# gear-genomics/tracy

Hardware: AMD Instinct MI355X
Metric: GCUPS (tracy align: Gotoh affine-gap DP cells per second, whole job) (higher is better)
Workload: dtype int16 (score sweeps) / int32 (tracebacks)

## Files before the change

### tracy_amd/csrc/pipe_kernels.h

```cpp
#ifndef TRACY_AMD_PIPE_KERNELS_H
#define TRACY_AMD_PIPE_KERNELS_H

#include <hip/hip_runtime.h>

#include "capi_internal.h"
#include "stream_plan.h"

namespace {
using namespace tracyhip;

__global__ __launch_bounds__(64) void trim_kernel(const uint8_t* __restrict__ ops, const uint64_t* __restrict__ ops_off,
                                                  const uint32_t* __restrict__ ops_len, const uint32_t* __restrict__ ref_len,
                                                  const uint8_t* __restrict__ forward, const uint32_t* __restrict__ trim_left,
                                                  const uint32_t* __restrict__ trim_right, uint32_t ntraces, TrimRec* __restrict__ out) {
  const uint32_t t = blockIdx.x;
  if (t >= ntraces) return;
  const uint8_t* o = ops + ops_off[t];
  const uint32_t L = ops_len[t];
  const uint32_t lane = threadIdx.x;
  int32_t s = -1, e = -1;
  for (uint32_t base = 0; base < L; base += 64) {
    const uint32_t j = base + lane;
    const bool hit = (j < L) && (o[L - 1 - j] != 'h');
    const unsigned long long m = __ballot(hit);
// ... 106 lines not shown
    float pr[5];
    for (int k = 0; k < 5; ++k) pr[k] = prof[d.off + (uint64_t)k * d.stride + r];
    int32_t best = INT32_MIN;
    for (uint32_t b = 0; b < 5; ++b) {
      const int32_t q = onehot_score(pr, b, fmatch, fmis);
      best = q > best ? q : best;
    }
    sum += best > 0 ? best : 0;
    sum1 += best > -1 ? best : -1;
  }
  for (int o = 32; o > 0; o >>= 1) { sum += __shfl_down(sum, o, 64); sum1 += __shfl_down(sum1, o, 64); }
  if (threadIdx.x == 0) {
    out[blockIdx.x] = sum;
    if (out1) out1[blockIdx.x] = sum1;
  }
}

constexpr uint32_t kCqBytesPerThread = 16;
__global__ void encode_cq_kernel(const uint8_t* __restrict__ in, uint8_t* __restrict__ out, uint64_t n, int32_t* flag, uint8_t* __restrict__ special) {
  const uint64_t i0 = ((uint64_t)blockIdx.x * blockDim.x + threadIdx.x) * kCqBytesPerThread;
  int32_t f = 0;
  if (i0 < n) {
    const uint32_t cnt = n - i0 < kCqBytesPerThread ? (uint32_t)(n - i0) : kCqBytesPerThread;
    uint8_t b[kCqBytesPerThread];
    if (cnt == kCqBytesPerThread) __builtin_memcpy(b, in + i0, kCqBytesPerThread);
    else for (uint32_t j = 0; j < cnt; ++j) b[j] = in[i0 + j];
    bool any = false;
#pragma unroll
    for (uint32_t j = 0; j < kCqBytesPerThread; ++j) {
      const uint32_t c = j < cnt ? cq_code(b[j]) : 0u;
      b[j] = (uint8_t)c;
      if (c >= 4u) { f |= c >= 5u ? 2 : 4; any = true; }
    }
    if (cnt == kCqBytesPerThread) __builtin_memcpy(out + i0, b, kCqBytesPerThread);
    else for (uint32_t j = 0; j < cnt; ++j) out[i0 + j] = b[j];
    if (any && special) { special[i0 >> 8] = 1; special[(i0 + cnt - 1) >> 8] = 1; }
  }
  if (f) atomicOr(flag, f);
}
__global__ void cq_rows_kernel(const uint8_t* __restrict__ in, uint64_t n, int32_t* flag) {
  const uint64_t i0 = ((uint64_t)blockIdx.x * blockDim.x + threadIdx.x) * kCqBytesPerThread;
  if (i0 >= n) return;
  const uint32_t cnt = n - i0 < kCqBytesPerThread ? (uint32_t)(n - i0) : kCqBytesPerThread;
  uint8_t b[kCqBytesPerThread];
  if (cnt == kCqBytesPerThread) __builtin_memcpy(b, in + i0, kCqBytesPerThread);
  else for (uint32_t j = 0; j < cnt; ++j) b[j] = in[i0 + j];
  bool bad = false;
#pragma unroll
  for (uint32_t j = 0; j < kCqBytesPerThread; ++j)
    if (j < cnt && !cq_row_char(b[j])) bad = true;
  if (bad) atomicOr(flag, 1);
}

__device__ __forceinline__ uint32_t encode_word(uint32_t w, uint32_t cnt, bool& any_special, bool& invalid) {
  uint32_t codes = 0;
#pragma unroll
  for (uint32_t j = 0; j < 4u; ++j) {
    const uint8_t ch = (uint8_t)(w >> (8 * j));
    const uint8_t up = ch & 0xdfu;
    const uint32_t c = up == 'A' ? 0u : up == 'C' ? 1u : up == 'G' ? 2u : up == 'T' ? 3u : up == 'N' ? 4u : 5u;
    if (j < cnt) {
      invalid |= !(ch == 'A' || ch == 'C' || ch == 'G' || ch == 'T' || ch == 'N');
      any_special |= c >= 4u;
    }
    codes |= c << (8 * j);
  }
  return codes;
}
__global__ __launch_bounds__(256) void encode_codes_kernel(const uint8_t* __restrict__ in, uint8_t* __restrict__ out, uint64_t n,
                                                           uint8_t* __restrict__ special, int32_t* __restrict__ verr) {
  const uint64_t i0 = ((uint64_t)blockIdx.x * blockDim.x + threadIdx.x) * 16u;
  if (i0 >= n) return;
  bool any_special = false, invalid = false;
  if (n - i0 >= 16u) {
    uint32_t w[4];
    __builtin_memcpy(w, in + i0, 16);
#pragma unroll
    for (int q = 0; q < 4; ++q) w[q] = encode_word(w[q], 4u, any_special, invalid);
    __builtin_memcpy(out + i0, w, 16);
  } else {
    for (uint64_t i = i0; i < n; i += 4) {
      const uint32_t cnt = (n - i < 4u) ? (uint32_t)(n - i) : 4u;
      uint32_t w = 0;
      for (uint32_t j = 0; j < cnt; ++j) w |= (uint32_t)in[i + j] << (8 * j);
      const uint32_t c = encode_word(w, cnt, any_special, invalid);
      for (uint32_t j = 0; j < cnt; ++j) out[i + j] = (uint8_t)(c >> (8 * j));
    }
  }
  if (any_special) special[i0 >> 8] = 1;
  if (verr && invalid) atomicOr(verr, 4);
}

struct VoteDesc { uint64_t a1_off, a2_off; uint32_t stride, m, n, pad; };
constexpr int kVoteK = 11;
constexpr uint32_t kVoteBits = 1u << 16;
constexpr uint32_t kVotePiece = 65, kVoteTile = 64 * kVotePiece;
__device__ inline uint32_t vote_hash(uint32_t kmer) { return (kmer * 0x9E3779B1u) >> 16; }
__global__ __launch_bounds__(64) void kmer_vote_kernel(const VoteDesc* __restrict__ desc, const float* __restrict__ prof,
                                                       const uint8_t* __restrict__ codes, uint32_t* __restrict__ votes) {
  __shared__ uint32_t bm[2][kVoteBits / 32];
  __shared__ uint8_t cons[1040];
  __shared__ __attribute__((aligned(16))) uint8_t win[kVoteTile + 16];
  const VoteDesc d = desc[blockIdx.x];
  const uint32_t lane = threadIdx.x;
  uint32_t hf = 0, hr = 0;
  const uint32_t m = d.m < 1024u ? d.m : 1024u;
  if (m >= (uint32_t)kVoteK && d.n >= (uint32_t)kVoteK) {
    for (uint32_t i = lane; i < kVoteBits / 32; i += 64) { bm[0][i] = 0; bm[1][i] = 0; }
    constexpr uint32_t kCols = 8;
    for (uint32_t j0 = 0; j0 < m; j0 += 64 * kCols) {
      float v[kCols][4];
#pragma unroll
      for (uint32_t u = 0; u < kCols; ++u) {
        const uint32_t j = j0 + 64 * u + lane, jc = j < m ? j : m - 1;
#pragma unroll
        for (uint32_t k = 0; k < 4; ++k) v[u][k] = prof[d.a1_off + (uint64_t)k * d.stride + jc];
      }
#pragma unroll
      for (uint32_t u = 0; u < kCols; ++u) {
        const uint32_t j = j0 + 64 * u + lane;
        uint32_t best = 0;
        float bv = v[u][0];
#pragma unroll
        for (uint32_t k = 1; k < 4; ++k) {
          const bool g = v[u][k] > bv;
          bv = g ? v[u][k] : bv;
          best = g ? k : best;
        }
        if (j < m) cons[j] = (uint8_t)best;
      }
    }
    __syncthreads();
// ... 64 lines not shown
```

### tracy_amd/csrc/pipeline.hip

```cpp
#include <hip/hip_runtime.h>

#include <algorithm>
#include <cstdlib>
#include <cstring>
#include <numeric>
#include <string>
#include <thread>
#include <vector>

#include "../../include/tracy_hip.h"
#include "capi_internal.h"
#include "launch.h"
#include "pipe_internal.h"
#include "pipe_kernels.h"
#include "stream_fields.h"

using namespace tracyhip;

namespace {
void reset_call_stats(tracyhip_ctx* ctx, uint32_t ntraces) {
  ctx->stats = tracyhip_call_stats{};
  ctx->stats.traces = ntraces;
  for (auto* l : ctx->lanes) l->stats = tracyhip_call_stats{};
}
// ... 689 lines not shown
  if ((rc = ctx_begin(ctx))) return rc;
  *empty = job->ntraces == 0;
  return TRACYHIP_OK;
}

static int align_traces_one(tracyhip_ctx* ctx, const tracyhip_align_job* job, const tracyhip_params* prm, int mem, const tracyhip_align_result* out) {
  bool empty = false;
  int rc = align_check_args(ctx, job, prm, mem, out, &empty);
  if (rc || empty) return rc;
  if (job->refs.kind == TRACYHIP_SEQ_PROFILE) return wildtype_align(ctx, job, prm, mem, out);
  rc = stream_align(ctx, job, prm, mem, out);
  if (rc != kStreamNo) return rc;
  return align_traces_legacy(ctx, job, prm, mem, out);
}

struct AlignRun {
  tracyhip_ctx* ctx;
  const tracyhip_align_job* job;
  const tracyhip_params* prm;
  const int mem;
  const tracyhip_align_result* out;
  const uint32_t nt;
  const tracyhip_seqset& sp;
  const tracyhip_seqset& sr;
  hipStream_t st;
  tracyhip_params p;
  const void *d_prof = nullptr, *d_ref = nullptr;
  int32_t* d_verr = nullptr;
  std::vector<uint32_t> mf, mt, tl, rn, ridx;
  const TrimSrc trims;
  std::vector<B16TableDesc> td;
  bool b16 = false;
  OrientOut oo;
  std::vector<TrimRec> h_trim;
  void *d_final_sc = nullptr, *d_ops = nullptr, *d_olen = nullptr;
  uint64_t ops_total = 0;

  AlignRun(tracyhip_ctx* c, const tracyhip_align_job* j, const tracyhip_params* q, int m, const tracyhip_align_result* o)
      : ctx(c), job(j), prm(q), mem(m), out(o), nt(j->ntraces), sp(j->profiles), sr(j->refs), st(c->stream), p(*q), trims(trims_of(j)) {
    p.hfree = 1;
    p.vfree = 0;
  }

  int setup() {
    int rc;
    const uint64_t ep = seqset_extent(sp), er = seqset_extent(sr);
    if ((rc = stage_in(ctx, ctx->dev[DB_IN1], sp.data, ep * 4, mem, &d_prof))) return rc;
    if ((rc = stage_in(ctx, ctx->dev[DB_IN2], sr.data, er, mem, &d_ref))) return rc;
    HIP_TRY(ctx->dev[DB_ERR].ensure(kErrBytes));
    HIP_TRY(hipMemsetAsync(ctx->dev[DB_ERR].p, 0, kErrBytes, st));
    d_verr = static_cast<int32_t*>(ctx->dev[DB_ERR].p) + kErrVerdictWord;
    HIP_TRY(ctx->ensure_codes(er ? er : 1, st));
    if (er) {
      hipLaunchKernelGGL(encode_codes_kernel, dim3((unsigned)((er + 4095) / 4096)), dim3(256), 0, st, static_cast<const uint8_t*>(d_ref),
                         ctx->codes(), er, ctx->special_blocks(), job->oriented ? (int32_t*)nullptr : d_verr);
      HIP_TRY(hipGetLastError());
    }
    mf.resize(nt); mt.resize(nt); tl.resize(nt); rn.resize(nt); ridx.resize(nt);
    uint64_t max_mn = 0;
    for (uint32_t t = 0; t < nt; ++t) {
      ridx[t] = job->ref_index ? job->ref_index[t] : t;
      if (ridx[t] >= sr.count) return set_error(TRACYHIP_ERR_ARG, "ref_index[%u] out of range", t);
      mf[t] = sp.length[t];
      rn[t] = sr.length[ridx[t]];
      uint32_t l = trims.left(t), r = trims.right(t);
      if ((uint64_t)l + r >= mf[t]) { l = 0; r = 0; }
      tl[t] = l;
      mt[t] = mf[t] - (l + r);
      max_mn = std::max<uint64_t>(max_mn, (uint64_t)mf[t] + rn[t]);
    }
    if ((rc = check_params(&p, max_mn))) return rc;

    return TRACYHIP_OK;
  }

  int orient() {
    int rc;
    std::vector<uint64_t> off1(nt);
    uint64_t tot1 = 0;
    for (uint32_t t = 0; t < nt; ++t) { off1[t] = tot1; tot1 += (uint64_t)mt[t] + rn[t]; }
    OrientIn oi{};
    HIP_TRY(ensure_into(ctx->dev[DB_PRELIM_OPS], tot1 ? tot1 : 1, oi.d_ops));
    HIP_TRY(ensure_into(ctx->dev[DB_PRELIM_OFF], nt, oi.d_ops_off));
    HIP_TRY(ensure_into(ctx->dev[DB_PRELIM_LEN], nt, oi.d_ops_len));
    HIP_TRY(ensure_into(ctx->dev[DB_PRELIM_SCORE], nt, oi.d_score));
    HIP_TRY(ctx->pin[PB_TMP].ensure(sizeof(uint64_t) * (size_t)nt + (size_t)nt * 16));
    std::memcpy(ctx->pin[PB_TMP].p, off1.data(), sizeof(uint64_t) * (size_t)nt);
    HIP_TRY(hipMemcpyAsync(ctx->dev[DB_PRELIM_OFF].p, ctx->pin[PB_TMP].p, sizeof(uint64_t) * (size_t)nt, hipMemcpyHostToDevice, st));
    std::vector<uint64_t> a1o(nt), a2o(nt);
    for (uint32_t t = 0; t < nt; ++t) { a1o[t] = sp.offset[t] + tl[t]; a2o[t] = sr.offset[ridx[t]]; }
    b16 = p.ge < 0 && p.go <= 0 && sub_limit(&p) <= kWideScore && !ctx->knobs.no_band16;
    if (b16) {
      td.resize(nt);
      for (uint32_t t = 0; t < nt; ++t) td[t] = B16TableDesc{sp.offset[t], 0, mf[t], mf[t], 0, 0};
      if ((rc = build_b16_tables(ctx, ctx->dev[DB_B16TAB_PROFILE], d_prof, false, td, &p))) return rc;
    }
    oi.nt = nt; oi.d_prof = d_prof; oi.a1_off = a1o.data(); oi.mf = mf.data(); oi.mt = mt.data(); oi.a2_off = a2o.data(); oi.rn = rn.data();
    oi.oriented = job->oriented; oi.exact = job->strand_by_certificate == 0; oi.d_verr = d_verr; oi.ends_only = true;
    if (b16) { oi.d_qp = static_cast<const int16_t*>(ctx->dev[DB_B16TAB_PROFILE].p); oi.td = td.data(); oi.row0 = tl.data(); }
    if ((rc = orient_and_align(ctx, p, oi, oo))) return rc;

    return TRACYHIP_OK;
  }

  int trim() {
    HIP_TRY(ctx->dev[DB_TRIMREC].ensure(sizeof(TrimRec) * (size_t)nt));
    HIP_TRY(ctx->dev[DB_TRIM_IN].ensure(3 * sizeof(uint32_t) * (size_t)nt + (size_t)nt));
// ... 512 lines not shown
      if ((uint64_t)(uint32_t)(TL + TR + 1) >= (uint64_t)mf[t]) { soff[t] = 0; sl[t] = mf[t]; }
      else { soff[t] = TL; sl[t] = mf[t] - TL - TR; }
      max_mn = std::max<uint64_t>(max_mn, (uint64_t)mf[t] + rn[t]);
      maxbc = std::max(maxbc, mf[t]);
      maxcol = std::max(maxcol, mt[t]);
    }
    if ((rc = check_params(&p, max_mn))) return rc;

    ep = seqset_extent(sp); er = seqset_extent(sr);
    for (uint32_t t = 0; t < nt; ++t) {
      if (!bc.peaks) sext = std::max<uint64_t>(sext, bc.signal_offset[t] + 4ull * bc.nsamples[t]);
      bext = std::max<uint64_t>(bext, bc.bc_offset[t] + bc.bc_len[t]);
    }
    if ((rc = stage_in(ctx, buf(), sp.data, ep * 4, mem, &d_prof))) return rc;
    if ((rc = stage_in(ctx, buf(), sr.data, er, mem, &d_ref))) return rc;
    if (wildtype && given && (rc = stage_in(ctx, buf(), srp.data, seqset_extent(srp) * 4, mem, &d_refprof))) return rc;
    if (wildtype && !given) {
      wt_rev_base = seqset_extent(srp);
      DevBuf& bw = buf();
      float* d_w; HIP_TRY(ensure_into(bw, std::max<uint64_t>(2 * wt_rev_base, 1), d_w));
      HIP_TRY(hipMemcpyAsync(d_w, srp.data, wt_rev_base * 4, mem == TRACYHIP_MEM_HOST ? hipMemcpyHostToDevice : hipMemcpyDeviceToDevice, st));
      std::vector<ProfSeq> hs(srp.count);
      for (uint32_t i = 0; i < srp.count; ++i) hs[i] = ProfSeq{srp.offset[i], srp.length[i], 0};
      const ProfSeq* ds;
      if ((rc = upload(ctx, buf(), hs, &ds))) return rc;
      HIP_TRY(launch_prof_revcomp(ds, srp.count, d_w, d_w, wt_rev_base, st));
      d_refprof = d_w;
    }
    if (bc.peaks) { if ((rc = stage_in(ctx, buf(), bc.peaks, bext * 16, mem, &d_peaks))) return rc; }
    else {
      if ((rc = stage_in(ctx, buf(), bc.signal, sext * 4, mem, &d_sig))) return rc;
      if ((rc = stage_in(ctx, buf(), bc.bcpos, bext * 4, mem, &d_pos))) return rc;
    }
    for (uint32_t t = 0; t < nt; ++t) dext = std::max<uint64_t>(dext, out->dcp_offset[t] + 2ull * dp.maxindel + 2);
    if ((rc = io(bc.primary, bext, true, &d_pri))) return rc;
    if ((rc = io(bc.secondary, bext, true, &d_sec))) return rc;
    if ((rc = io(out->bp, sizeof(BreakpointOut) * (size_t)nt, false, &d_bp))) return rc;
    if ((rc = io(out->secdecomp, bext, false, &d_sd))) return rc;
    if ((rc = io(out->fractions, sizeof(double) * 2 * (size_t)nt, false, &d_fr))) return rc;
    if ((rc = io(out->dcp_indel, dext * 4, false, &d_di))) return rc;
    if ((rc = io(out->dcp_err, dext * 4, false, &d_de))) return rc;
    if (mem == TRACYHIP_MEM_HOST) {
      HIP_TRY(hipMemsetAsync(d_di, 0, dext * 4, st));
      HIP_TRY(hipMemsetAsync(d_de, 0, dext * 4, st));
    }
    if ((rc = io(out->dstatus, sizeof(DecompOut) * (size_t)nt, false, &d_dst))) return rc;
    if ((rc = io(out->score_trim, sizeof(int32_t) * (size_t)nt, false, &d_strim))) return rc;

    HIP_TRY(ctx->dev[DB_ERR].ensure(kErrBytes));
    HIP_TRY(hipMemsetAsync(ctx->dev[DB_ERR].p, 0, kErrBytes, st));
    HIP_TRY(ctx->ensure_codes(er ? er : 1, st));
    if (er) {
      int32_t* d_verr = static_cast<int32_t*>(ctx->dev[DB_ERR].p) + kErrVerdictWord;
      hipLaunchKernelGGL(encode_codes_kernel, dim3((unsigned)((er + 4095) / 4096)), dim3(256), 0, st, static_cast<const uint8_t*>(d_ref),
                         ctx->codes(), er, ctx->special_blocks(), job->oriented ? (int32_t*)nullptr : d_verr);
      HIP_TRY(hipGetLastError());
      int32_t herr = 0;
      HIP_TRY(hipMemcpyAsync(&herr, d_verr, sizeof(int32_t), hipMemcpyDeviceToHost, st));
      HIP_TRY(ctx_sync(ctx));
      if ((herr & 4) && !wildtype) return set_error(TRACYHIP_ERR_ARG, "reference windows must be upper-case [ACGTN] (loadSingleFasta, fasta.h:54-95)");
    }

    return TRACYHIP_OK;
  }

  int orientation() {
    int rc;
    stage_clock.mark("decompose.2_orientation");
    HIP_TRY(b_sc2.ensure(sizeof(int32_t) * 2 * (size_t)nt));
    h_sc2.assign(2 * (size_t)nt, 0);
    if (!given && !shared_stages) {
      DpProblem pb;
      DpProblemLease lease(ctx, pb);
      pb.mode = MODE_PROF; pb.a1_profile = true; pb.a2_profile = true; pb.d_a1 = d_prof; pb.d_a2 = d_refprof;
      pb.desc.resize(2 * (size_t)nt); pb.k.resize(2 * (size_t)nt);
      for (uint32_t t = 0; t < nt; ++t) {
        PairDesc d = qp_desc(t, true);
        d.a2_off = srp.offset[ridx[t]];
        pb.desc[t] = d;
        d.out = nt + t; d.a2_off += wt_rev_base;
        pb.desc[nt + t] = d;
        pb.k[t] = pb.k[nt + t] = choose_k(d.m, MODE_PROF);
      }
      if ((rc = run_dp(ctx, pb, &p, false, false, static_cast<int32_t*>(b_sc2.p), nullptr, nullptr, nullptr))) return rc;
      HIP_TRY(hipMemcpy(h_sc2.data(), b_sc2.p, sizeof(int32_t) * 2 * (size_t)nt, hipMemcpyDeviceToHost));
    }
    h_fwd.assign(nt, 0); h_rc.assign(nt, 0);
    if (!shared_stages)
      for (uint32_t t = 0; t < nt; ++t) {
        if (given) { h_fwd[t] = job->oriented[t] ? 1 : 0; h_rc[t] = 0; }
        else { h_fwd[t] = h_sc2[t] > h_sc2[nt + t] ? 1 : 0; h_rc[t] = !h_fwd[t]; }
      }

    return TRACYHIP_OK;
  }

  int gotoh_rows() {
    int rc;
    stage_clock.mark("decompose.3_gotoh");
    off1.resize(nt);
    for (uint32_t t = 0; t < nt; ++t) { off1[t] = tot1; tot1 += (uint64_t)mt[t] + rn[t]; }
    HIP_TRY(b_ops1.ensure(tot1 ? tot1 : 1));
    HIP_TRY(b_len1.ensure(sizeof(uint32_t) * (size_t)nt));
    HIP_TRY(b_r0.ensure(tot1 ? tot1 : 1));
    HIP_TRY(b_r1.ensure(tot1 ? tot1 : 1));
    if ((rc = upload(ctx, buf(), off1, &d_off1))) return rc;
    if (shared_stages) {
// ... 838 lines not shown
```

### tracy_amd/csrc/stream.hip

```cpp
#include <hip/hip_runtime.h>

#include <algorithm>
#include <cstring>
#include <numeric>
#include <string>
#include <type_traits>
#include <vector>

#include "../../include/tracy_hip.h"
#include "capi_internal.h"
#include "decompose_launch.h"
#include "launch.h"
#include "pipe_internal.h"
#include "pipe_kernels.h"
#include "stream_fields.h"
#include "stream_plan.h"

using namespace tracyhip;

#define TRY(expr) do { const int _rc = (expr); if (_rc) return _rc; } while (0)

namespace {

struct Arena {
// ... 198 lines not shown
    d.a2_off = G.ref_off; d.n = G.rn; d.a2_stride = G.rn;
    d.out = t;
    d.flags = S.rc ? PAIR_A2_REVCOMP : 0u;
    desc_trim[t] = d;
  }
  });
}

__global__ void s_prelim_plan_kernel(SParams p, int mode, int early, const SGeom* __restrict__ geom, STrace* __restrict__ tr, const uint32_t* __restrict__ d_ce,
                                     const int32_t* __restrict__ top, uint32_t* __restrict__ dead, PairDesc* __restrict__ cand,
                                     uint8_t* __restrict__ kc, int prio) {
  wave_prio(prio);
  const uint32_t t = blockIdx.x * blockDim.x + threadIdx.x;
  if (t >= p.nt) return;
  kc[t] = 0;
  STrace S = tr[t];
  if (((S.mark & ST_EARLY) != 0u) != (early != 0)) return;
  if (dead[t]) return;
  const SGeom G = geom[t];
  const bool from_front = S.cls == 0 && S.rc == S.g;
  const uint32_t ce = from_front ? S.ce : d_ce[t];
  S.ce = ce;
  uint32_t dd = 0;
  if (ce == 0u) dd = SD_JUNK;
  else {
    const SubWindow sw = s_sub_window(G.mt, ce, top[t], S.sstar, p.ge);
    S.gap = (uint32_t)(sw.g < 0x7fffffff ? sw.g : 0x7fffffff);
    S.shift = sw.a;
    int K = sw.K;
    if (K && mode == 0 && !b16_origin_ok(p.match, p.mismatch, p.go, p.ge, G.mt, sw.n)) K = 0;
    if (K && !s_fits_lds(sw.n, K)) K = 0;
    if (!K) dd = SD_PRELIM_BAND;
    else if (sw.n > p.ncap) dd = SD_SHAPE;
    else {
      PairDesc q{};
      q.a1_off = G.tab_off + G.tl;
      q.a1_stride = G.tab_stride;
      q.m = G.mt;
      q.n = sw.n;
      q.a2_stride = sw.n;
      q.a2_off = G.ref_off + (S.rc ? (uint64_t)(G.rn - ce) : (uint64_t)sw.a);
      q.flags = S.rc ? PAIR_A2_REVCOMP : 0u;
      q.out = t;
      q.ckpt_off = band_pack(sw.dlo, sw.dhi);
      q.lastrow_off = mode == 0 ? 0ull : ((uint64_t)(G.rn - ce) | ((uint64_t)sw.a << 32));
      cand[t] = q;
      kc[t] = (uint8_t)K;
    }
  }
  tr[t] = S;
  if (dd) dead[t] |= dd;
}

constexpr uint32_t kScanBlock = 256, kScanTop = 1024;
struct ScanPart { uint32_t n[4]; unsigned long long bytes; };
__device__ __forceinline__ int s_bucket(int K, const PairDesc& d, int quads) {
  return K == 12 ? 0 : K == 8 ? 1 : (quads && b16_narrow_ok(band_dmin(d), band_dmax(d))) ? 3 : 2;
}
__device__ __forceinline__ unsigned long long s_word_bytes(const PairDesc& d, int K, int kind, unsigned long long* words = nullptr) {
  if (words) *words = b16_words(d.m, d.n, K, band_dmin(d), band_dmax(d));
  return kind == 0 ? ((b16_store_words(d.m, d.n, K, band_dmin(d), band_dmax(d)) * b16_word_bytes(K) + 15ull) & ~15ull) : 0ull;
}
__global__ __launch_bounds__(kScanBlock) void s_scan_partial_kernel(const PairDesc* __restrict__ cand, const uint8_t* __restrict__ kc, uint32_t n, int kind,
                                                                    int quads, ScanPart* __restrict__ part, int prio) {
  wave_prio(prio);
  __shared__ uint32_t s_n[4];
  __shared__ unsigned long long s_b;
  if (threadIdx.x < 4) s_n[threadIdx.x] = 0;
  if (threadIdx.x == 4) s_b = 0;
  __syncthreads();
  const uint32_t i = blockIdx.x * kScanBlock + threadIdx.x;
  const int K = i < n ? kc[i] : 0;
  if (K) {
    const PairDesc d = cand[i];
    atomicAdd(&s_n[s_bucket(K, d, quads)], 1u);
    if (kind == 0) atomicAdd(&s_b, s_word_bytes(d, K, kind));
  }
  __syncthreads();
  if (threadIdx.x == 0) part[blockIdx.x] = ScanPart{{s_n[0], s_n[1], s_n[2], s_n[3]}, s_b};
}
__global__ __launch_bounds__(kScanTop) void s_scan_top_kernel(ScanPart* __restrict__ part, uint32_t nb, uint32_t* __restrict__ count,
                                                              unsigned long long* __restrict__ stat, int prio) {
  wave_prio(prio);
  __shared__ uint32_t s_n[4][kScanTop];
  __shared__ unsigned long long s_b[kScanTop];
  const uint32_t tid = threadIdx.x;
  const uint32_t per = (nb + kScanTop - 1) / kScanTop;
  const uint32_t lo = tid * per < nb ? tid * per : nb, hi = lo + per < nb ? lo + per : nb;
  uint32_t c[4] = {0, 0, 0, 0};
  unsigned long long bytes = 0;
  for (uint32_t i = lo; i < hi; ++i) { for (int b = 0; b < 4; ++b) c[b] += part[i].n[b]; bytes += part[i].bytes; }
  for (int b = 0; b < 4; ++b) s_n[b][tid] = c[b];
  s_b[tid] = bytes;
  __syncthreads();
  for (uint32_t d = 1; d < kScanTop; d <<= 1) {
    uint32_t v[4] = {0, 0, 0, 0};
    unsigned long long vb = 0;
    if (tid >= d) { for (int b = 0; b < 4; ++b) v[b] = s_n[b][tid - d]; vb = s_b[tid - d]; }
    __syncthreads();
    for (int b = 0; b < 4; ++b) s_n[b][tid] += v[b];
    s_b[tid] += vb;
    __syncthreads();
  }
  uint32_t at[4];
  for (int b = 0; b < 4; ++b) at[b] = s_n[b][tid] - c[b];
  unsigned long long off = s_b[tid] - bytes;
  for (uint32_t i = lo; i < hi; ++i) {
    const ScanPart x = part[i];
    part[i] = ScanPart{{at[0], at[1], at[2], at[3]}, off};
    for (int b = 0; b < 4; ++b) at[b] += x.n[b];
    off += x.bytes;
  }
  if (tid == 0)
    for (int b = 0; b < 4; ++b) {
      count[b] = s_n[b][kScanTop - 1];
      stat[SB_LIST + b] += s_n[b][kScanTop - 1];
    }
}
__global__ __launch_bounds__(kScanBlock) void s_scan_place_kernel(PairDesc* __restrict__ cand, uint8_t* __restrict__ kc, uint32_t n, uint32_t unit_mod, int kind,
                                                                  int quads, unsigned long long cap_bytes, const ScanPart* __restrict__ part, uint32_t* __restrict__ idx,
                                                                  uint32_t* __restrict__ dead, unsigned long long* __restrict__ stat, int prio) {
  wave_prio(prio);
  __shared__ uint32_t s_n[4][kScanBlock];
  __shared__ unsigned long long s_b[kScanBlock];
  __shared__ unsigned long long s_stat[SB_LIST];
  const uint32_t tid = threadIdx.x;
  if (tid < SB_LIST) s_stat[tid] = 0;
  const uint32_t i = blockIdx.x * kScanBlock + tid;
  const int K = i < n ? kc[i] : 0;
  PairDesc d{};
  unsigned long long words = 0, mine = 0;
  if (K) { d = cand[i]; mine = s_word_bytes(d, K, kind, &words); }
  const int bucket = K ? s_bucket(K, d, quads) : -1;
  for (int b = 0; b < 4; ++b) s_n[b][tid] = bucket == b ? 1u : 0u;
  s_b[tid] = mine;
  __syncthreads();
  for (uint32_t dd = 1; dd < kScanBlock; dd <<= 1) {
    uint32_t v[4] = {0, 0, 0, 0};
    unsigned long long vb = 0;
    if (tid >= dd) { for (int b = 0; b < 4; ++b) v[b] = s_n[b][tid - dd]; vb = s_b[tid - dd]; }
    __syncthreads();
    for (int b = 0; b < 4; ++b) s_n[b][tid] += v[b];
    s_b[tid] += vb;
    __syncthreads();
  }
  if (K) {
    const ScanPart base = part[blockIdx.x];
    const int b = bucket;
    const uint32_t pos = base.n[b] + s_n[b][tid] - 1u;
    const unsigned long long off = base.bytes + s_b[tid] - mine;
    idx[(size_t)b * n + pos] = i;
    if (off + mine > cap_bytes) {
      kc[i] = 0;
      cand[i].flags = d.flags | PAIR_SKIP;
      atomicOr(dead + (i % unit_mod), SD_MEM);
    } else {
      cand[i].bits_off = off;
      atomicAdd(&s_stat[0], words * (unsigned long long)K);
      atomicAdd(&s_stat[1], (kind == 0 ? words * b16_word_bytes(K) : 0ull) + 12ull * d.m + d.n + 4ull);
      atomicAdd(&s_stat[2], mine);
      atomicAdd(&s_stat[SB_HIST + s_width_bucket(band_dmin(d), band_dmax(d))], 1ull);
    }
  }
  __syncthreads();
  if (tid < SB_LIST && s_stat[tid]) atomicAdd(stat + tid, s_stat[tid]);
}

__global__ void s_align_final_plan_kernel(SParams p, int early, const SGeom* __restrict__ geom, STrace* __restrict__ tr, const uint32_t* __restrict__ ends,
                                          uint32_t* __restrict__ dead, PairDesc* __restrict__ cand, uint8_t* __restrict__ kc,
                                          unsigned long long* __restrict__ cnt, int prio) {
  wave_prio(prio);
  with_counters(cnt, [&](unsigned long long* lc) {
  const uint32_t t = blockIdx.x * blockDim.x + threadIdx.x;
  if (t >= p.nt) return;
  kc[t] = 0;
  STrace S = tr[t];
  if (((S.mark & ST_EARLY) != 0u) != (early != 0)) return;
  if (dead[t]) return;
  const SGeom G = geom[t];
  const uint32_t lead = ends[2 * t] + S.shift, ce = ends[2 * t + 1] + S.shift;
  S.trim = s_trim_finish(lead, ce >= lead ? ce - lead : 0u, G.rn, G.rl, G.rr, S.fwd != 0);
  s_count(lc, SC_PRELIM_BANDED);
  if (early) S.mark |= ST_COUNTED_PRELIM;
  const uint32_t m = G.mf, n = S.trim.len;
  const SFinalBand fb = s_final_band(m, n, s_final_width(S.gap));
  uint32_t dd = 0;
  if (!fb.K) dd = SD_FINAL_BAND;
  else if (n > p.ncap) dd = SD_SHAPE;
  else {
    S.bw = (int32_t)fb.w;
    PairDesc q{};
    q.a1_off = G.tab_off;
    q.a1_stride = G.tab_stride;
    q.m = m;
    q.n = n;
    q.a2_stride = n;
    q.a2_off = G.ref_off + (S.rc ? G.rn - S.trim.ri - S.trim.len : S.trim.ri);
    q.flags = S.rc ? PAIR_A2_REVCOMP : 0u;
    q.out = t;
    q.ckpt_off = band_pack(fb.dlo, fb.dhi);
    cand[t] = q;
    kc[t] = (uint8_t)fb.K;
    s_count(lc, SC_FINAL_BANDED);
    if (early) S.mark |= ST_COUNTED_FINAL;
  }
  tr[t] = S;
  if (dd) dead[t] |= dd;
  });
}

struct AlignOutDev {
  int32_t *score_fwd, *score_rev, *score_prelim, *score_final;
  uint8_t* forward;
  uint32_t *slice_begin, *slice_len, *ref_pos, *ops_len;
};
__global__ void s_align_finish_kernel(SParams p, const STrace* __restrict__ tr, const int32_t* __restrict__ top_full, uint32_t* __restrict__ dead,
                                      AlignOutDev o, unsigned long long* __restrict__ cnt) {
  with_counters(cnt, [&](unsigned long long* lc) {
// ... 243 lines not shown
  if (i >= n || !fo0[i].ok) return;
  fo1[i] = fo0[i];
  fs1[i] = fs0[i];
  fe1[2 * i] = fe0[2 * i];
  fe1[2 * i + 1] = fe0[2 * i + 1];
}
int front_tiers_run_wide(tracyhip_ctx* ctx, const tracyhip_params& p, StreamCommon& sc, uint32_t n, const int16_t* d_qp, const uint8_t* d_codes,
                         const uint32_t* d_row, uint32_t max_rest, bool after_quads) {
  const bool lists = !ctx->knobs.no_front_lists && n >= ctx->knobs.front_list_min;
  if (lists) HIP_TRY(hipMemsetAsync(sc.fcount, 0, 2 * sizeof(uint32_t), ctx->stream));
  const bool list1 = lists && after_quads;
  if (list1) HIP_TRY(front_list(ctx, n, sc.fo0, sc.flist, sc.fcount, sc.fo1));
  int rc = front_tier(ctx, p, sc.fd, n, d_qp, d_codes, d_row, 8, 60, max_rest, sc.fpairs1, sc.fo1, sc.fs1, sc.fe1, after_quads ? sc.fo0 : nullptr,
                      list1 ? sc.flist : nullptr, list1 ? sc.fcount : nullptr);
  if (rc) return rc;
  if (after_quads) {
    hipLaunchKernelGGL(s_front_fold_kernel, dim3((n + 255) / 256), dim3(256), 0, ctx->stream, n, sc.fo0, sc.fs0, sc.fe0, sc.fo1, sc.fs1, sc.fe1, queued_prio(ctx, 1));
    HIP_TRY(hipGetLastError());
  }
  if (lists) HIP_TRY(front_list(ctx, n, sc.fo1, sc.flist, sc.fcount + 1, sc.fo2));
  return front_tier(ctx, p, sc.fd, n, d_qp, d_codes, d_row, kFrontK, kFrontHalfW, max_rest, sc.fpairs2, sc.fo2, sc.fs2, sc.fe2, sc.fo1,
                    lists ? sc.flist : nullptr, lists ? sc.fcount + 1 : nullptr);
}
constexpr int32_t kQuadHalfW = 5;

int front_tiers_run(tracyhip_ctx* ctx, const tracyhip_params& p, StreamCommon& sc, uint32_t n, const int16_t* d_qp, const uint8_t* d_codes, const uint32_t* d_row,
                    uint32_t max_rest) {
  const bool quads = !ctx->knobs.no_quads && n >= ctx->knobs.quad_tier_min;
  int rc = TRACYHIP_OK;
  if (quads) rc = front_tier(ctx, p, sc.fd, n, d_qp, d_codes, d_row, 0, kQuadHalfW, max_rest, sc.fpairs0, sc.fo0, sc.fs0, sc.fe0, nullptr, nullptr, nullptr);
  if (rc == kStreamNo && quads) return front_tiers_run_wide(ctx, p, sc, n, d_qp, d_codes, d_row, max_rest, false);
  if (rc) return rc;
  return front_tiers_run_wide(ctx, p, sc, n, d_qp, d_codes, d_row, max_rest, quads);
}

struct BandLaunch {
  int kind = 0;
  const int16_t* qp = nullptr;
  const uint8_t* codes = nullptr;
  int32_t* scores = nullptr;
  uint32_t* ends = nullptr;
  uint8_t* ops = nullptr;
  const uint64_t* ops_off = nullptr;
  uint32_t* ops_len = nullptr;
  uint32_t code_cap = 0;
  int hfree = 1;
};
int band_stage(tracyhip_ctx* ctx, const tracyhip_params& p, StreamCommon& sc, uint32_t n, uint32_t unit_mod, int stage_no, const BandLaunch& bl, uint64_t cap_bytes) {
  hipStream_t st = ctx->stream;
  uint32_t* count = sc.count + 4 * stage_no;
  const uint32_t nb = (n + kScanBlock - 1) / kScanBlock;
  const int quads = (!ctx->knobs.no_quads && b16_quad_lds(bl.code_cap) <= 64u * 1024u) ? 1 : 0;
  const int prio = queued_prio(ctx, 2);
  hipLaunchKernelGGL(s_scan_partial_kernel, dim3(nb), dim3(kScanBlock), 0, st, sc.cand, sc.kc, n, bl.kind, quads, sc.part, prio);
  hipLaunchKernelGGL(s_scan_top_kernel, dim3(1), dim3(kScanTop), 0, st, sc.part, nb, count, sc.bstat + SB_COUNT * stage_no, prio);
  hipLaunchKernelGGL(s_scan_place_kernel, dim3(nb), dim3(kScanBlock), 0, st, sc.cand, sc.kc, n, unit_mod, bl.kind, quads, (unsigned long long)cap_bytes, sc.part, sc.idx, sc.dead,
                     sc.bstat + SB_COUNT * stage_no, prio);
  HIP_TRY(hipGetLastError());
  Band16Args a{};
  a.prio = prio;
  a.pairs = sc.cand; a.npairs = n; a.qp = bl.qp; a.codes = bl.codes; a.bits = static_cast<uint8_t*>(ctx->dev[DB_BITS].p); a.scores = bl.scores; a.ends = bl.ends;
  a.err = static_cast<int32_t*>(ctx->dev[DB_ERR].p); a.go = p.go; a.ge = p.ge; a.hfree = bl.hfree;
  a.ops = bl.ops; a.ops_off = bl.ops_off; a.ops_len = bl.ops_len; a.code_cap = bl.code_cap;
  Band16Args ak[4] = {a, a, a, a};
  for (int b = 0; b < 4; ++b) { ak[b].index = sc.idx + (size_t)b * n; ak[b].count = count + b; }
  if (!quads) ak[3].npairs = 0;
  TRY(timing_begin(ctx, bl.kind == 0 ? TRACYHIP_TIMER_TRACE : TRACYHIP_TIMER_ORIGIN, 0, 0));
  bool large = false;
  HIP_TRY(launch_band16_counted(bl.kind, ak[0], ak[1], ak[2], ak[3], st, (ctx->b16_fork_ok && !ctx->knobs.no_fork) ? &ctx->b16_fork : nullptr,
                                ctx->knobs.b16_multi_max, &large));
  if (large) ++sc.large_stages;
  TRY(timing_end(ctx));
  return TRACYHIP_OK;
}

uint64_t band_words_cap(uint64_t rows, uint64_t npairs, uint64_t budget_left) {
  const uint64_t worst = rows * 131 + npairs * 10240;
  return std::max<uint64_t>(std::min(worst, budget_left / 2), 1ull << 20);
}
struct OrientStage {
  const void* d_prof;
  const int16_t* d_qp;
  int32_t* d_lastrow;
  bool exact;
  PairDesc* desc_trim;
  std::function<int()> filler;
  std::function<int()> early_tail;
};
int queue_orientation(tracyhip_ctx* ctx, const tracyhip_params& p, const SParams& sp, const StreamHost& h, StreamCommon& sc, const OrientStage& os) {
  hipStream_t st = ctx->stream;
  const uint32_t nt = h.nt;
  const dim3 g256((nt + 255) / 256), b256(256);
  const float* prof = static_cast<const float*>(os.d_prof);
  hipLaunchKernelGGL(s_expand_kernel, g256, b256, 0, st, sc.geom, nt, sc.vd, sc.rm_rest, sc.rm_trim, sc.rm_full, sc.td);
  HIP_TRY(hipGetLastError());
  const bool prep_fork = ctx->b16_fork_ok && !ctx->knobs.no_fork;
  hipStream_t sp1 = st;
  if (prep_fork) {
    HIP_TRY(hipEventRecord(ctx->b16_fork.forked, st));
    HIP_TRY(hipStreamWaitEvent(ctx->b16_fork.side[1], ctx->b16_fork.forked, 0));
    sp1 = ctx->b16_fork.side[1];
    ctx->stream = sp1;
  }
  {
    int rc = timing_begin(ctx, TRACYHIP_TIMER_MISC, 0, h.tab_tot * 2);
    hipError_t e = hipSuccess;
    if (!rc) {
      e = launch_b16_tables(sc.td, nt, os.d_prof, false, p.match, p.mismatch, sub_limit(&p), kTagShift, const_cast<int16_t*>(os.d_qp),
                            static_cast<int32_t*>(ctx->dev[DB_ERR].p), sp1);
// ... 303 lines not shown
}
template <class Fields, class Result, class Out>
int copy_back_all(hipStream_t st, uint32_t nt, const Result& user, Out& o) {
  int rc = TRACYHIP_OK;
  Fields::each(user, o, [&](auto& u, auto& d, uint32_t per) {
    if (rc == TRACYHIP_OK) rc = copy_to_host(st, u, d, sizeof(*d) * per * (size_t)nt);
  });
  return rc;
}

struct StreamCall {
  tracyhip_ctx* ctx;
  const tracyhip_params* prm;
  const int mem;
  const CtxKnobs& kn;
  const uint32_t nt;
  const tracyhip_seqset &sp, &sr;
  hipStream_t st;
  tracyhip_params p;
  const TrimSrc trims;
  const bool exact, host;
  StreamHost& h;
  SGeom* geom = nullptr;
  uint32_t ncap = 0;
  uint64_t words_cap = 0;
  SParams spm{};
  dim3 g256, b256;
  const int16_t* d_qp = nullptr;
  int32_t* d_lastrow = nullptr;
  ReadBack rb;
  std::vector<uint32_t> dl;
  std::vector<uint64_t> sub_poff;
  std::vector<uint32_t> sub_plen, sub_ridx, sub_tl, sub_tr;

  template <class Job>
  StreamCall(tracyhip_ctx* c, const Job* j, const tracyhip_params* q, int m, StreamHost& h_)
      : ctx(c), prm(q), mem(m), kn(c->knobs), nt(j->ntraces), sp(j->profiles), sr(j->refs), st(c->stream), p(*q), trims(trims_of(j)),
        exact(j->strand_by_certificate == 0), host(m == TRACYHIP_MEM_HOST), h(h_), g256((j->ntraces + 255) / 256), b256(256) {
    p.hfree = 1;
    p.vfree = 0;
  }

  int size_ncap() {
    ncap = (h.maxmf + 200u + 7u) & ~3u;
    return 4ull * ncap + b16_table_bytes(12) > 64u * 1024u ? kStreamNo : TRACYHIP_OK;
  }

  int encode_references(const uint8_t* refs, uint64_t er) {
    HIP_TRY(ctx->dev[DB_ERR].ensure(kErrBytes));
    HIP_TRY(hipMemsetAsync(ctx->dev[DB_ERR].p, 0, kErrBytes, st));
    int32_t* d_verr = static_cast<int32_t*>(ctx->dev[DB_ERR].p) + kErrVerdictWord;
    HIP_TRY(ctx->ensure_codes(er ? er : 1, st));
    if (er) {
      hipLaunchKernelGGL(encode_codes_kernel, dim3((unsigned)((er + 4095) / 4096)), dim3(256), 0, st, refs, ctx->codes(), er, ctx->special_blocks(), d_verr);
      HIP_TRY(hipGetLastError());
    }
    return TRACYHIP_OK;
  }

  int upload_records(StreamCommon& sc, void* d_own, size_t own_bytes) {
    HIP_TRY(hipMemcpyAsync(sc.geom, geom, sizeof(SGeom) * (size_t)nt, hipMemcpyHostToDevice, st));
    HIP_TRY(hipMemcpyAsync(d_own, geom + nt, own_bytes, hipMemcpyHostToDevice, st));
    HIP_TRY(hipMemsetAsync(sc.dead, 0, sizeof(uint32_t) * (size_t)nt, st));
    HIP_TRY(hipMemsetAsync(sc.cnt, 0, sizeof(unsigned long long) * SC_COUNT, st));
    HIP_TRY(hipMemsetAsync(sc.bstat, 0, sizeof(unsigned long long) * SB_COUNT * 8, st));
    sc.large_stages = 0;
    return TRACYHIP_OK;
  }

  void fill_params() {
    spm.match = p.match; spm.mismatch = p.mismatch; spm.go = p.go; spm.ge = p.ge; spm.nt = nt; spm.exact = exact ? 1u : 0u; spm.ncap = ncap - 8u;
    spm.use_votes = 1u;
    spm.split_prefix = kn.sweeps_alone ? 1u : 0u;
    d_qp = static_cast<const int16_t*>(ctx->dev[DB_B16TAB_PROFILE].p);
    d_lastrow = static_cast<int32_t*>(ctx->dev[DB_LASTROW].p);
  }

  template <class GiveUp>
  int await_verdict(GiveUp give_up) {
    HIP_TRY(ctx_sync(ctx));
    timing_collect(ctx);
    if (rb.herr[kErrVerdictWord] & 4) {
      (void)give_up(kStreamNo);
      return set_error(TRACYHIP_ERR_ARG, "reference windows must be upper-case [ACGTN] (loadSingleFasta, fasta.h:54-95)");
    }
    return give_up(stream_range_verdict(p, rb.herr, h));
  }

  template <size_t NS, size_t NR>
  void list_dead(const char* what, const StreamCommon& sc, const int (&stage_timer)[NS], const DeadReason (&reasons)[NR]) {
    stats_from_counters(ctx, rb.hcnt, rb.hbst, (int)NS, stage_timer, sc.large_stages);
    ctx->stats.stream_ordered = 1;
    dl.clear();
    for (uint32_t t = 0; t < nt; ++t)
      if (rb.hdead[t]) dl.push_back(t);
    ctx->stats.fallback_traces += (uint32_t)dl.size();
    if (kn.verbose) {
      std::string why;
      for (const DeadReason& r : reasons) {
        uint32_t n = 0;
        for (uint32_t t : dl) n += (rb.hdead[t] & r.bit) != 0u;
        why += (why.empty() ? "" : ", ") + std::string(r.name) + " " + std::to_string(n);
      }
      fprintf(stderr, "stream-ordered %s: %u traces, %zu to the host-planned tiers (%s)\n", what, nt, dl.size(), why.c_str());
    }
  }

  template <class Job>
  void sub_job(Job& j, const void* d_prof, const void* d_ref) {
    const uint32_t nd = (uint32_t)dl.size();
    sub_poff.resize(nd); sub_plen.resize(nd); sub_ridx.resize(nd); sub_tl.resize(nd); sub_tr.resize(nd);
    for (uint32_t i = 0; i < nd; ++i) {
      const uint32_t t = dl[i];
      sub_poff[i] = sp.offset[t]; sub_plen[i] = sp.length[t]; sub_ridx[i] = h.ridx[t];
      sub_tl[i] = trims.left(t); sub_tr[i] = trims.right(t);
    }
    j.ntraces = nd;
    j.profiles.data = d_prof; j.profiles.offset = sub_poff.data(); j.profiles.length = sub_plen.data(); j.profiles.count = nd;
// ... 986 lines not shown
```

Baseline: 19040.

## Use wave-level ballots/shuffles for bucket scan and widen reference encoding per thread

```diff
diff --git a/tracy_amd/csrc/pipe_kernels.h b/tracy_amd/csrc/pipe_kernels.h
--- a/tracy_amd/csrc/pipe_kernels.h
+++ b/tracy_amd/csrc/pipe_kernels.h
@@ -182,32 +182,30 @@
   if (bad) atomicOr(flag, 1);
 }
 
+__device__ __forceinline__ uint32_t encode_code(uint32_t ch) {
+  const uint32_t up = ch & 0xdfu;
+  return up == 'A' ? 0u : up == 'C' ? 1u : up == 'G' ? 2u : up == 'T' ? 3u : up == 'N' ? 4u : 5u;
+}
 __device__ __forceinline__ uint32_t encode_word(uint32_t w, uint32_t cnt, bool& any_special, bool& invalid) {
-  uint32_t codes = 0;
-#pragma unroll
-  for (uint32_t j = 0; j < 4u; ++j) {
-    const uint8_t ch = (uint8_t)(w >> (8 * j));
-    const uint8_t up = ch & 0xdfu;
-    const uint32_t c = up == 'A' ? 0u : up == 'C' ? 1u : up == 'G' ? 2u : up == 'T' ? 3u : up == 'N' ? 4u : 5u;
-    if (j < cnt) {
-      invalid |= !(ch == 'A' || ch == 'C' || ch == 'G' || ch == 'T' || ch == 'N');
-      any_special |= c >= 4u;
-    }
-    codes |= c << (8 * j);
-  }
+  const uint32_t codes = encode_code(w & 0xffu) | (encode_code((w >> 8) & 0xffu) << 8) | (encode_code((w >> 16) & 0xffu) << 16) | (encode_code(w >> 24) << 24);
+  const uint32_t m = cnt >= 4u ? 0xffffffffu : (1u << (8u * cnt)) - 1u;
+  any_special |= (codes & 0x04040404u & m) != 0u;
+  invalid |= (((codes & (codes >> 2) & 0x01010101u) | (w & 0x20202020u)) & m) != 0u;
   return codes;
 }
-__global__ __launch_bounds__(256) void encode_codes_kernel(const uint8_t* __restrict__ in, uint8_t* __restrict__ out, uint64_t n,
-                                                           uint8_t* __restrict__ special, int32_t* __restrict__ verr) {
-  const uint64_t i0 = ((uint64_t)blockIdx.x * blockDim.x + threadIdx.x) * 16u;
+constexpr uint32_t kEncodeBytes = 64, kEncodeBlock = 256;
+inline unsigned encode_codes_grid(uint64_t n) { return (unsigned)((n + (uint64_t)kEncodeBytes * kEncodeBlock - 1) / ((uint64_t)kEncodeBytes * kEncodeBlock)); }
+__global__ __launch_bounds__(kEncodeBlock) void encode_codes_kernel(const uint8_t* __restrict__ in, uint8_t* __restrict__ out, uint64_t n,
+                                                                    uint8_t* __restrict__ special, int32_t* __restrict__ verr) {
+  const uint64_t i0 = ((uint64_t)blockIdx.x * blockDim.x + threadIdx.x) * kEncodeBytes;
   if (i0 >= n) return;
   bool any_special = false, invalid = false;
-  if (n - i0 >= 16u) {
-    uint32_t w[4];
-    __builtin_memcpy(w, in + i0, 16);
-#pragma unroll
-    for (int q = 0; q < 4; ++q) w[q] = encode_word(w[q], 4u, any_special, invalid);
-    __builtin_memcpy(out + i0, w, 16);
+  if (n - i0 >= kEncodeBytes) {
+    uint32_t w[kEncodeBytes / 4];
+    __builtin_memcpy(w, in + i0, kEncodeBytes);
+#pragma unroll
+    for (uint32_t q = 0; q < kEncodeBytes / 4; ++q) w[q] = encode_word(w[q], 4u, any_special, invalid);
+    __builtin_memcpy(out + i0, w, kEncodeBytes);
   } else {
     for (uint64_t i = i0; i < n; i += 4) {
       const uint32_t cnt = (n - i < 4u) ? (uint32_t)(n - i) : 4u;
diff --git a/tracy_amd/csrc/pipeline.hip b/tracy_amd/csrc/pipeline.hip
--- a/tracy_amd/csrc/pipeline.hip
+++ b/tracy_amd/csrc/pipeline.hip
@@ -765,7 +765,7 @@
     d_verr = static_cast<int32_t*>(ctx->dev[DB_ERR].p) + kErrVerdictWord;
     HIP_TRY(ctx->ensure_codes(er ? er : 1, st));
     if (er) {
-      hipLaunchKernelGGL(encode_codes_kernel, dim3((unsigned)((er + 4095) / 4096)), dim3(256), 0, st, static_cast<const uint8_t*>(d_ref),
+      hipLaunchKernelGGL(encode_codes_kernel, dim3(encode_codes_grid(er)), dim3(kEncodeBlock), 0, st, static_cast<const uint8_t*>(d_ref),
                          ctx->codes(), er, ctx->special_blocks(), job->oriented ? (int32_t*)nullptr : d_verr);
       HIP_TRY(hipGetLastError());
     }
@@ -1384,7 +1384,7 @@
     HIP_TRY(ctx->ensure_codes(er ? er : 1, st));
     if (er) {
       int32_t* d_verr = static_cast<int32_t*>(ctx->dev[DB_ERR].p) + kErrVerdictWord;
-      hipLaunchKernelGGL(encode_codes_kernel, dim3((unsigned)((er + 4095) / 4096)), dim3(256), 0, st, static_cast<const uint8_t*>(d_ref),
+      hipLaunchKernelGGL(encode_codes_kernel, dim3(encode_codes_grid(er)), dim3(kEncodeBlock), 0, st, static_cast<const uint8_t*>(d_ref),
                          ctx->codes(), er, ctx->special_blocks(), job->oriented ? (int32_t*)nullptr : d_verr);
       HIP_TRY(hipGetLastError());
       int32_t herr = 0;
diff --git a/tracy_amd/csrc/stream.hip b/tracy_amd/csrc/stream.hip
--- a/tracy_amd/csrc/stream.hip
+++ b/tracy_amd/csrc/stream.hip
@@ -274,7 +274,7 @@
   if (dd) dead[t] |= dd;
 }
 
-constexpr uint32_t kScanBlock = 256, kScanTop = 1024;
+constexpr uint32_t kScanBlock = 256, kScanWave = 64, kScanRounds = kScanBlock / kScanWave;
 struct ScanPart { uint32_t n[4]; unsigned long long bytes; };
 __device__ __forceinline__ int s_bucket(int K, const PairDesc& d, int quads) {
   return K == 12 ? 0 : K == 8 ? 1 : (quads && b16_narrow_ok(band_dmin(d), band_dmax(d))) ? 3 : 2;
@@ -283,109 +283,125 @@
   if (words) *words = b16_words(d.m, d.n, K, band_dmin(d), band_dmax(d));
   return kind == 0 ? ((b16_store_words(d.m, d.n, K, band_dmin(d), band_dmax(d)) * b16_word_bytes(K) + 15ull) & ~15ull) : 0ull;
 }
-__global__ __launch_bounds__(kScanBlock) void s_scan_partial_kernel(const PairDesc* __restrict__ cand, const uint8_t* __restrict__ kc, uint32_t n, int kind,
-                                                                    int quads, ScanPart* __restrict__ part, int prio) {
+__device__ __forceinline__ unsigned long long s_wave_sum(unsigned long long v) {
+  for (int o = 32; o > 0; o >>= 1) v += __shfl_down(v, o, 64);
+  return v;
+}
+template <class T>
+__device__ __forceinline__ T s_wave_scan(T v, uint32_t lane) {
+  for (uint32_t o = 1; o < 64u; o <<= 1) {
+    const T u = __shfl_up(v, o, 64);
+    if (lane >= o) v += u;
+  }
+  return v;
+}
+__global__ __launch_bounds__(kScanWave) void s_scan_partial_kernel(const PairDesc* __restrict__ cand, const uint8_t* __restrict__ kc, uint32_t n, int kind,
+                                                                   int quads, ScanPart* __restrict__ part, int prio) {
   wave_prio(prio);
-  __shared__ uint32_t s_n[4];
-  __shared__ unsigned long long s_b;
-  if (threadIdx.x < 4) s_n[threadIdx.x] = 0;
-  if (threadIdx.x == 4) s_b = 0;
-  __syncthreads();
-  const uint32_t i = blockIdx.x * kScanBlock + threadIdx.x;
-  const int K = i < n ? kc[i] : 0;
-  if (K) {
-    const PairDesc d = cand[i];
-    atomicAdd(&s_n[s_bucket(K, d, quads)], 1u);
-    if (kind == 0) atomicAdd(&s_b, s_word_bytes(d, K, kind));
-  }
-  __syncthreads();
-  if (threadIdx.x == 0) part[blockIdx.x] = ScanPart{{s_n[0], s_n[1], s_n[2], s_n[3]}, s_b};
-}
-__global__ __launch_bounds__(kScanTop) void s_scan_top_kernel(ScanPart* __restrict__ part, uint32_t nb, uint32_t* __restrict__ count,
-                                                              unsigned long long* __restrict__ stat, int prio) {
-  wave_prio(prio);
-  __shared__ uint32_t s_n[4][kScanTop];
-  __shared__ unsigned long long s_b[kScanTop];
-  const uint32_t tid = threadIdx.x;
-  const uint32_t per = (nb + kScanTop - 1) / kScanTop;
-  const uint32_t lo = tid * per < nb ? tid * per : nb, hi = lo + per < nb ? lo + per : nb;
+  const uint32_t lane = threadIdx.x;
   uint32_t c[4] = {0, 0, 0, 0};
   unsigned long long bytes = 0;
-  for (uint32_t i = lo; i < hi; ++i) { for (int b = 0; b < 4; ++b) c[b] += part[i].n[b]; bytes += part[i].bytes; }
-  for (int b = 0; b < 4; ++b) s_n[b][tid] = c[b];
-  s_b[tid] = bytes;
-  __syncthreads();
-  for (uint32_t d = 1; d < kScanTop; d <<= 1) {
-    uint32_t v[4] = {0, 0, 0, 0};
-    unsigned long long vb = 0;
-    if (tid >= d) { for (int b = 0; b < 4; ++b) v[b] = s_n[b][tid - d]; vb = s_b[tid - d]; }
-    __syncthreads();
-    for (int b = 0; b < 4; ++b) s_n[b][tid] += v[b];
-    s_b[tid] += vb;
-    __syncthreads();
-  }
-  uint32_t at[4];
-  for (int b = 0; b < 4; ++b) at[b] = s_n[b][tid] - c[b];
-  unsigned long long off = s_b[tid] - bytes;
-  for (uint32_t i = lo; i < hi; ++i) {
-    const ScanPart x = part[i];
-    part[i] = ScanPart{{at[0], at[1], at[2], at[3]}, off};
-    for (int b = 0; b < 4; ++b) at[b] += x.n[b];
-    off += x.bytes;
-  }
-  if (tid == 0)
+#pragma unroll
+  for (uint32_t r = 0; r < kScanRounds; ++r) {
+    const uint32_t i = blockIdx.x * kScanBlock + r * kScanWave + lane;
+    const int K = i < n ? kc[i] : 0;
+    int bucket = -1;
+    if (K) {
+      const PairDesc d = cand[i];
+      bucket = s_bucket(K, d, quads);
+      if (kind == 0) bytes += s_word_bytes(d, K, kind);
+    }
+    for (int b = 0; b < 4; ++b) c[b] += (uint32_t)__popcll(__ballot(bucket == b));
+  }
+  if (kind == 0) bytes = s_wave_sum(bytes);
+  if (lane == 0) part[blockIdx.x] = ScanPart{{c[0], c[1], c[2], c[3]}, bytes};
+}
+__global__ __launch_bounds__(kScanWave) void s_scan_top_kernel(ScanPart* __restrict__ part, uint32_t nb, uint32_t* __restrict__ count,
+                                                               unsigned long long* __restrict__ stat, int prio) {
+  wave_prio(prio);
+  const uint32_t lane = threadIdx.x;
+  uint32_t at[4] = {0, 0, 0, 0};
+  unsigned long long off = 0;
+  const ScanPart none{{0, 0, 0, 0}, 0};
+  ScanPart next = lane < nb ? part[lane] : none;
+  for (uint32_t i0 = 0; i0 < nb; i0 += kScanWave) {
+    const uint32_t i = i0 + lane;
+    const ScanPart x = next;
+    next = (i + kScanWave < nb) ? part[i + kScanWave] : none;
+    ScanPart y;
+    for (int b = 0; b < 4; ++b) y.n[b] = s_wave_scan(x.n[b], lane);
+    y.bytes = s_wave_scan(x.bytes, lane);
+    if (i < nb) part[i] = ScanPart{{at[0] + y.n[0] - x.n[0], at[1] + y.n[1] - x.n[1], at[2] + y.n[2] - x.n[2], at[3] + y.n[3] - x.n[3]}, off + y.bytes - x.bytes};
+    for (int b = 0; b < 4; ++b) at[b] += __shfl(y.n[b], 63, 64);
+    off += __shfl(y.bytes, 63, 64);
+  }
+  if (lane == 0)
     for (int b = 0; b < 4; ++b) {
-      count[b] = s_n[b][kScanTop - 1];
-      stat[SB_LIST + b] += s_n[b][kScanTop - 1];
-    }
-}
-__global__ __launch_bounds__(kScanBlock) void s_scan_place_kernel(PairDesc* __restrict__ cand, uint8_t* __restrict__ kc, uint32_t n, uint32_t unit_mod, int kind,
-                                                                  int quads, unsigned long long cap_bytes, const ScanPart* __restrict__ part, uint32_t* __restrict__ idx,
-                                                                  uint32_t* __restrict__ dead, unsigned long long* __restrict__ stat, int prio) {
+      count[b] = at[b];
+      stat[SB_LIST + b] += at[b];
+    }
+}
+__global__ __launch_bounds__(kScanWave) void s_scan_place_kernel(PairDesc* __restrict__ cand, uint8_t* __restrict__ kc, uint32_t n, uint32_t unit_mod, int kind,
+                                                                 int quads, unsigned long long cap_bytes, const ScanPart* __restrict__ part, uint32_t* __restrict__ idx,
+                                                                 uint32_t* __restrict__ dead, unsigned long long* __restrict__ stat, int prio) {
   wave_prio(prio);
-  __shared__ uint32_t s_n[4][kScanBlock];
-  __shared__ unsigned long long s_b[kScanBlock];
-  __shared__ unsigned long long s_stat[SB_LIST];
-  const uint32_t tid = threadIdx.x;
-  if (tid < SB_LIST) s_stat[tid] = 0;
-  const uint32_t i = blockIdx.x * kScanBlock + tid;
-  const int K = i < n ? kc[i] : 0;
-  PairDesc d{};
-  unsigned long long words = 0, mine = 0;
-  if (K) { d = cand[i]; mine = s_word_bytes(d, K, kind, &words); }
-  const int bucket = K ? s_bucket(K, d, quads) : -1;
-  for (int b = 0; b < 4; ++b) s_n[b][tid] = bucket == b ? 1u : 0u;
-  s_b[tid] = mine;
-  __syncthreads();
-  for (uint32_t dd = 1; dd < kScanBlock; dd <<= 1) {
-    uint32_t v[4] = {0, 0, 0, 0};
-    unsigned long long vb = 0;
-    if (tid >= dd) { for (int b = 0; b < 4; ++b) v[b] = s_n[b][tid - dd]; vb = s_b[tid - dd]; }
-    __syncthreads();
-    for (int b = 0; b < 4; ++b) s_n[b][tid] += v[b];
-    s_b[tid] += vb;
-    __syncthreads();
-  }
-  if (K) {
-    const ScanPart base = part[blockIdx.x];
-    const int b = bucket;
-    const uint32_t pos = base.n[b] + s_n[b][tid] - 1u;
-    const unsigned long long off = base.bytes + s_b[tid] - mine;
-    idx[(size_t)b * n + pos] = i;
-    if (off + mine > cap_bytes) {
-      kc[i] = 0;
-      cand[i].flags = d.flags | PAIR_SKIP;
-      atomicOr(dead + (i % unit_mod), SD_MEM);
-    } else {
-      cand[i].bits_off = off;
-      atomicAdd(&s_stat[0], words * (unsigned long long)K);
-      atomicAdd(&s_stat[1], (kind == 0 ? words * b16_word_bytes(K) : 0ull) + 12ull * d.m + d.n + 4ull);
-      atomicAdd(&s_stat[2], mine);
-      atomicAdd(&s_stat[SB_HIST + s_width_bucket(band_dmin(d), band_dmax(d))], 1ull);
-    }
-  }
-  __syncthreads();
-  if (tid < SB_LIST && s_stat[tid]) atomicAdd(stat + tid, s_stat[tid]);
+  const uint32_t lane = threadIdx.x;
+  const unsigned long long below = (1ull << lane) - 1ull;
+  ScanPart base = part[blockIdx.x];
+  unsigned long long st_cells = 0, st_bytes = 0, st_words = 0, st_hist = 0;
+  int Ks[kScanRounds];
+  PairDesc ds[kScanRounds];
+#pragma unroll
+  for (uint32_t r = 0; r < kScanRounds; ++r) {
+    const uint32_t i = blockIdx.x * kScanBlock + r * kScanWave + lane;
+    Ks[r] = i < n ? kc[i] : 0;
+    ds[r] = PairDesc{};
+    if (Ks[r]) ds[r] = cand[i];
+  }
+#pragma unroll
+  for (uint32_t r = 0; r < kScanRounds; ++r) {
+    const uint32_t i = blockIdx.x * kScanBlock + r * kScanWave + lane;
+    const int K = Ks[r];
+    const PairDesc d = ds[r];
+    unsigned long long words = 0, mine = 0;
+    if (K) mine = s_word_bytes(d, K, kind, &words);
+    const int bucket = K ? s_bucket(K, d, quads) : -1;
+    uint32_t before = 0;
+    for (int b = 0; b < 4; ++b) {
+      const unsigned long long mb = __ballot(bucket == b);
+      if (bucket == b) before = base.n[b] + (uint32_t)__popcll(mb & below);
+      base.n[b] += (uint32_t)__popcll(mb);
+    }
+    const unsigned long long upto = s_wave_scan(mine, lane);
+    const unsigned long long off = base.bytes + upto - mine;
+    base.bytes += __shfl(upto, 63, 64);
+    int wb = -1;
+    if (K) {
+      idx[(size_t)bucket * n + before] = i;
+      if (off + mine > cap_bytes) {
+        kc[i] = 0;
+        cand[i].flags = d.flags | PAIR_SKIP;
+        atomicOr(dead + (i % unit_mod), SD_MEM);
+      } else {
+        cand[i].bits_off = off;
+        st_cells += words * (unsigned long long)K;
+        st_bytes += (kind == 0 ? words * b16_word_bytes(K) : 0ull) + 12ull * d.m + d.n + 4ull;
+        st_words += mine;
+        wb = s_width_bucket(band_dmin(d), band_dmax(d));
+      }
+    }
+    for (int hb = 0; hb < SB_HIST_N; ++hb) {
+      const unsigned long long mh = __ballot(wb == hb);
+      if ((int)lane == hb) st_hist += (unsigned long long)__popcll(mh);
+    }
+  }
+  st_cells = s_wave_sum(st_cells); st_bytes = s_wave_sum(st_bytes); st_words = s_wave_sum(st_words);
+  if (lane == 0) {
+    if (st_cells) atomicAdd(stat + SB_CELLS, st_cells);
+    if (st_bytes) atomicAdd(stat + SB_BYTES, st_bytes);
+    if (st_words) atomicAdd(stat + SB_WORDS, st_words);
+  }
+  if (lane < (uint32_t)SB_HIST_N && st_hist) atomicAdd(stat + SB_HIST + lane, st_hist);
 }
 
 __global__ void s_align_final_plan_kernel(SParams p, int early, const SGeom* __restrict__ geom, STrace* __restrict__ tr, const uint32_t* __restrict__ ends,
@@ -735,9 +751,9 @@
   const uint32_t nb = (n + kScanBlock - 1) / kScanBlock;
   const int quads = (!ctx->knobs.no_quads && b16_quad_lds(bl.code_cap) <= 64u * 1024u) ? 1 : 0;
   const int prio = queued_prio(ctx, 2);
-  hipLaunchKernelGGL(s_scan_partial_kernel, dim3(nb), dim3(kScanBlock), 0, st, sc.cand, sc.kc, n, bl.kind, quads, sc.part, prio);
-  hipLaunchKernelGGL(s_scan_top_kernel, dim3(1), dim3(kScanTop), 0, st, sc.part, nb, count, sc.bstat + SB_COUNT * stage_no, prio);
-  hipLaunchKernelGGL(s_scan_place_kernel, dim3(nb), dim3(kScanBlock), 0, st, sc.cand, sc.kc, n, unit_mod, bl.kind, quads, (unsigned long long)cap_bytes, sc.part, sc.idx, sc.dead,
+  hipLaunchKernelGGL(s_scan_partial_kernel, dim3(nb), dim3(kScanWave), 0, st, sc.cand, sc.kc, n, bl.kind, quads, sc.part, prio);
+  hipLaunchKernelGGL(s_scan_top_kernel, dim3(1), dim3(kScanWave), 0, st, sc.part, nb, count, sc.bstat + SB_COUNT * stage_no, prio);
+  hipLaunchKernelGGL(s_scan_place_kernel, dim3(nb), dim3(kScanWave), 0, st, sc.cand, sc.kc, n, unit_mod, bl.kind, quads, (unsigned long long)cap_bytes, sc.part, sc.idx, sc.dead,
                      sc.bstat + SB_COUNT * stage_no, prio);
   HIP_TRY(hipGetLastError());
   Band16Args a{};
@@ -1147,7 +1163,7 @@
     int32_t* d_verr = static_cast<int32_t*>(ctx->dev[DB_ERR].p) + kErrVerdictWord;
     HIP_TRY(ctx->ensure_codes(er ? er : 1, st));
     if (er) {
-      hipLaunchKernelGGL(encode_codes_kernel, dim3((unsigned)((er + 4095) / 4096)), dim3(256), 0, st, refs, ctx->codes(), er, ctx->special_blocks(), d_verr);
+      hipLaunchKernelGGL(encode_codes_kernel, dim3(encode_codes_grid(er)), dim3(kEncodeBlock), 0, st, refs, ctx->codes(), er, ctx->special_blocks(), d_verr);
       HIP_TRY(hipGetLastError());
     }
     return TRACYHIP_OK;
@@ -1157,8 +1173,9 @@
     HIP_TRY(hipMemcpyAsync(sc.geom, geom, sizeof(SGeom) * (size_t)nt, hipMemcpyHostToDevice, st));
     HIP_TRY(hipMemcpyAsync(d_own, geom + nt, own_bytes, hipMemcpyHostToDevice, st));
     HIP_TRY(hipMemsetAsync(sc.dead, 0, sizeof(uint32_t) * (size_t)nt, st));
-    HIP_TRY(hipMemsetAsync(sc.cnt, 0, sizeof(unsigned long long) * SC_COUNT, st));
-    HIP_TRY(hipMemsetAsync(sc.bstat, 0, sizeof(unsigned long long) * SB_COUNT * 8, st));
+    char* const c0 = reinterpret_cast<char*>(sc.cnt);
+    char* const c1 = reinterpret_cast<char*>(sc.bstat + SB_COUNT * 8);
+    HIP_TRY(hipMemsetAsync(c0, 0, (size_t)(c1 - c0), st));
     sc.large_stages = 0;
     return TRACYHIP_OK;
   }
```

Measured after the change: 19150, median of 4. No clear change (+0.6%).
